# mfkiwl/msckf_stereo_c

Hardware: AMD Instinct MI355X
Metric: stereo frames/sec/node on EuRoC-shape input; ATE RMSE vs CPU ref (higher is better)
Workload: dtype f64

## Files before the change

### msckf_stereo_c_amd/csrc/abi/mskf_capi_ekf.cpp

```cpp
#include <algorithm>
#include <chrono>
#include <cmath>
#include <cstring>
#include "../../../include/mskf_chi2_table.h"
#include "mskf_internal.h"

namespace {
constexpr int kMaxRows = 65536;

size_t align_up(size_t v, size_t a) { return (v + a - 1) / a * a; }

int dev_alloc(double **p, size_t n, hipStream_t st) {
    MSKF_HIPCHK(hipMalloc((void **)p, n * sizeof(double)));
    MSKF_HIPCHK(hipMemsetAsync(*p, 0, n * sizeof(double), st));
    return MSKF_OK;
}
}

struct EkfExtra {
    EkfStreamDev desc_static;
    bool desc_valid = false;
    double *P_alt = nullptr;
    std::vector<double *> retired_hs;
};
// ... 377 lines not shown
    unsigned long long clone_mask = 0ULL;
    bool pairs = a.n_feat > 0, wave = a.n_feat > 0;
    int pair_a = -1, pair_b = -1, frows_cls[3] = {0, 0, 0};
    for (int j = 0; j < a.n_feat; ++j) {
        const mskf_ekf_feature &f = a.features[j];
        L.n_tri += f.needs_init ? 1 : 0;
        if (f.n_obs < 2 || f.n_obs > E.max_clones || f.obs_start < 0 || f.obs_start + f.n_obs > a.n_obs) return MSKF_ERR_INVALID;
        if (f.needs_init && (f.n_init < 1 || f.n_init > E.max_clones || f.init_start < 0 || f.init_start + f.n_init > a.n_obs)) return MSKF_ERR_INVALID;
        if (f.n_obs != 2) pairs = false;
        else if (pairs) {
            const int c0 = a.obs_clone[f.obs_start], c1 = a.obs_clone[f.obs_start + 1];
            if (j == 0) { pair_a = c0; pair_b = c1; }
            if (!(c0 < c1) || c0 != pair_a || c1 != pair_b) pairs = false;
        }
        if (f.n_obs > FEAT_WAVE_CLONES || (f.needs_init && f.n_init > TRI_SMALL_CLONES)) wave = false;
        L.m_total += 4 * f.n_obs - 3;
        B.max_frows = std::max(B.max_frows, 4 * f.n_obs);
        const int cls = std::max(f.n_obs, f.needs_init ? f.n_init : 0) <= FEAT_SMALL_CLONES ? 1 : 2;
        frows_cls[cls] = std::max(frows_cls[cls], 4 * f.n_obs);
        ++L.cnt[cls];
        for (int o = 0; o < f.n_obs; ++o) {
            const int c = a.obs_clone[f.obs_start + o];
            if (c < 0 || c >= a.n_clones) return MSKF_ERR_INVALID;
            clone_mask |= 1ULL << c;
        }
        const double nj = 4.0 * f.n_obs - 3.0, M = f.n_obs, dd = E.d;
        B.fl_feat += 2.0 * nj * (4.0 * M) * (6.0 * M) + 2.0 * nj * dd * dd + 2.0 * nj * nj * dd;
    }
    if (L.m_total > kMaxRows) { mskf_set_error("stacked Jacobian exceeds the row capacity"); return MSKF_ERR_CAPACITY; }
    L.clones = B.in_bytes;
    L.feats = align_up(L.clones + sizeof(mskf_clone_state) * (size_t)a.n_clones, 16);
    L.obs_clone = align_up(L.feats + sizeof(EkfFeatDev) * (size_t)a.n_feat, 16);
    L.obs_z = align_up(L.obs_clone + sizeof(int) * (size_t)a.n_obs, 16);
    L.tri = align_up(L.obs_z + sizeof(double) * 4 * (size_t)a.n_obs, 16);
// ... 71 lines not shown
        }
    for (int i = 0; i < n; ++i) {
        const mskf_ekf_update_args &a = args[i];
        const EkfUpdatePlan &L = plan[i];
        if (a.n_clones) std::memcpy(hin + L.clones, a.clones, sizeof(mskf_clone_state) * (size_t)a.n_clones);
        EkfFeatDev *fd = (EkfFeatDev *)(hin + L.feats);
        int *tri = (int *)(hin + L.tri);
        int n_tri_w = 0, row = 0;
        for (int j = 0; j < a.n_feat; ++j) {
            const mskf_ekf_feature &f = a.features[j];
            fd[j].obs_start = f.obs_start; fd[j].n_obs = f.n_obs;
            fd[j].needs_init = f.needs_init; fd[j].init_start = f.init_start; fd[j].n_init = f.n_init;
            fd[j].row_off = row;
            fd[j].position[0] = f.position[0]; fd[j].position[1] = f.position[1]; fd[j].position[2] = f.position[2];
            fd[j].colmask = 0ULL;
            row += 4 * f.n_obs - 3;
            if (f.needs_init) tri[n_tri_w++] = j;
        }
        if (a.n_obs) {
            std::memcpy(hin + L.obs_clone, a.obs_clone, sizeof(int) * (size_t)a.n_obs);
            std::memcpy(hin + L.obs_z, a.obs_z, sizeof(double) * 4 * (size_t)a.n_obs);
        }
        EkfStreamDev &D = ctx->ekf_desc.h[i];
        base_desc(streams[i], D);
        D.n_clones = a.n_clones; D.n_feat = a.n_feat; D.n_obs = a.n_obs;
        D.route = L.route; D.na_max = L.na_max;
        D.dof_offset = a.dof_offset; D.apply_row_cap = a.apply_row_cap;
        D.m_total = L.m_total;
        for (int k = 0; k < 3; ++k) D.gravity[k] = a.gravity[k];
        D.clones = (const mskf_clone_state *)(din + L.clones);
        D.feats = (EkfFeatDev *)(din + L.feats);
// ... 272 lines not shown
```

### msckf_stereo_c_amd/csrc/hip/ekf_cap.h

```cpp
#pragma once
#include "ekf_device.h"

struct EkfCapResult {
    int stacked;
    int end;
    int na;
    unsigned long long clones;
};

__device__ __forceinline__ int ekf_act_column(unsigned long long clones, int i) {
    int q = i / 6;
    unsigned long long m = clones;
    while (q-- > 0) m &= m - 1;
    return EKF_IMU_DIM + 6 * (int)__builtin_ctzll(m) + i % 6;
}

template <int NT = 256>
__device__ __forceinline__ EkfCapResult ekf_cap_local(const EkfStreamDev &S, bool publish) {
    __shared__ int s_sum[NT], s_cross[NT];
    __shared__ unsigned long long s_or[NT / 64];
    __shared__ int s_cap_from, s_tot[2];
    __shared__ unsigned long long s_mask;
    const int tid = threadIdx.x, nf = S.n_feat;
    const int per = (nf + NT - 1) / NT;
    const int j0 = tid * per, j1 = min(nf, j0 + per);
    __syncthreads();
    int local = 0;
    for (int j = j0; j < j1; ++j) if (S.feat_status[j] & 2) local += 4 * S.feats[j].n_obs - 3;
    s_sum[tid] = local;
    __syncthreads();
    for (int off = 1; off < NT; off <<= 1) {
        const int v = tid >= off ? s_sum[tid - off] : 0;
        __syncthreads();
        s_sum[tid] += v;
        __syncthreads();
    }
    const int before = s_sum[tid] - local;
    int cross = nf;
    if (S.apply_row_cap) {
        int run = before;
        for (int j = j0; j < j1; ++j)
            if (S.feat_status[j] & 2) { run += 4 * S.feats[j].n_obs - 3; if (run > S.max_stack_rows) { cross = j; break; } }
    }
    s_cross[tid] = cross;
    __syncthreads();
    if (tid == 0) {
        int c = nf;
        for (int t = 0; t < NT; ++t) if (s_cross[t] < c) c = s_cross[t];
        s_cap_from = c < nf ? c + 1 : nf;
    }
    __syncthreads();
    const int cap_from = s_cap_from;
    int stack = 0, meff = 0;
    unsigned long long orm = 0ULL;
    for (int j = j0; j < j1; ++j) {
        EkfFeatDev &F = S.feats[j];
        const int n = 4 * F.n_obs - 3;
        const bool pass = (S.feat_status[j] & 2) != 0;
        if (pass && j < cap_from) { stack += n; meff = F.row_off + n; orm |= F.colmask; }
        else if (pass && publish) {
            F.colmask = 0ULL; S.feat_status[j] &= (uint8_t)~2;
            for (int i = 0; i < n; ++i) S.rowmask[F.row_off + i] = 0ULL;
        }
    }
    __syncthreads();
    s_sum[tid] = stack; s_cross[tid] = meff;
    for (int off = 32; off > 0; off >>= 1) orm |= __shfl_xor(orm, off);
    if ((tid & 63) == 0) s_or[tid >> 6] = orm;
    __syncthreads();
    if (tid == 0) {
        int st = 0, me = 0;
        for (int t = 0; t < NT; ++t) { st += s_sum[t]; if (s_cross[t] > me) me = s_cross[t]; }
        unsigned long long m = 0ULL;
        for (int w = 0; w < NT / 64; ++w) m |= s_or[w];
// ... 19 lines not shown
```

### msckf_stereo_c_amd/csrc/hip/ekf_kernels.hip

```cpp
#include <mutex>
#include <type_traits>
#include "ekf_device.h"
#include "ekf_meas.h"
#include "chol_block.h"

using namespace ekf;

#define WG 256

__device__ __forceinline__ double wave_sum(double v) {
    for (int off = 32; off > 0; off >>= 1) v += __shfl_xor(v, off);
    return v;
}

__device__ __forceinline__ double block_sum(double v, double *s_red) {
    v = wave_sum(v);
    const int nw = blockDim.x >> 6;
    __syncthreads();
    if ((threadIdx.x & 63) == 0) s_red[threadIdx.x >> 6] = v;
    __syncthreads();
    double t = 0;
    for (int i = 0; i < nw; ++i) t += s_red[i];
    return t;
}
// ... 335 lines not shown

#define GATE_LDS_ROWS 120
__device__ __forceinline__ size_t pk(int i, int j) { return (size_t)i * (i + 1) / 2 + j; }
template <int MAXC, bool WAVE, int TPB>
__global__ __launch_bounds__(TPB, 2) void k_ekf_feature_blocks(const EkfStreamDev *streams, const int *work, int n_work, int lds_rows, int arena_doubles, int cls_lo, int cls_hi) {
    constexpr int GS = WAVE ? 64 : TPB;
    constexpr int NSUB = TPB / GS;
    const int gt = WAVE ? (int)(threadIdx.x & 63) : (int)threadIdx.x;
    const int sub = WAVE ? (int)(threadIdx.x >> 6) : 0;
    const int item = (int)blockIdx.x * NSUB + sub;
    if (item >= n_work) return;
    const int wcode = work[item];
    const int w_slot = (wcode >> 8) & 0xff, w_nslots = wcode & 0xff;
    const EkfStreamDev &S = streams[wcode >> 16];
    const int d = S.d, ld = S.ld;
    constexpr int BLK_DOUBLES = (12 + 24 + 4 + 12) * MAXC + 3 * (6 * MAXC + 1);
    constexpr int PAN_RS = WAVE ? 16 : ((4 * MAXC + 15) / 16) * 16;
    static_assert(WAVE || BLK_DOUBLES >= LNB * PAN_RS, "panel does not fit the dead scratch");
    __shared__ double s_blk_all[NSUB][BLK_DOUBLES];
    double *s_blk = s_blk_all[sub];
    double (*sHf)[3] = reinterpret_cast<double (*)[3]>(s_blk);
    double (*sHx)[6] = reinterpret_cast<double (*)[6]>(s_blk + 12 * MAXC);
    double *sr = s_blk + 36 * MAXC;
    double (*sV)[4 * MAXC] = reinterpret_cast<double (*)[4 * MAXC]>(s_blk + 40 * MAXC);
    double (*sCoef)[3] = reinterpret_cast<double (*)[3]>(s_blk + 52 * MAXC);
    __shared__ CholBlockShared s_cb;
    __shared__ double sBeta_all[NSUB][3], sVV_all[NSUB][3];
    __shared__ int sObsOfClone_all[NSUB][MAX_CLONES_DEV];
    __shared__ int sCloneOfObs_all[NSUB][MAXC];
    extern __shared__ double s_arena_all[];
    double *s_arena = s_arena_all + (size_t)sub * arena_doubles;
    typedef typename std::conditional<WAVE, TriScratchT<2 * TRI_SMALL_CLONES>,
                                      typename std::conditional<(MAXC <= FEAT_SMALL_CLONES), TriScratchT<2 * MAXC>, TriScratch>::type>::type TriT;
    TriT &sTri = *reinterpret_cast<TriT *>(s_arena);
    __shared__ double sW_all[NSUB][4 * MAXC];
    __shared__ double sRo_all[NSUB][4 * MAXC];
    __shared__ double sPos_all[NSUB][3];
    __shared__ int sValid_all[NSUB];
    __shared__ double sRed[8];
    double *sBeta = sBeta_all[sub], *sVV = sVV_all[sub], *sW = sW_all[sub], *sPos = sPos_all[sub], *sRo = sRo_all[sub];
    int *sObsOfClone = sObsOfClone_all[sub], *sCloneOfObs = sCloneOfObs_all[sub];
    int &sValid = sValid_all[sub];
    auto GSYNC = [&]() {
        if (WAVE) { __builtin_amdgcn_wave_barrier(); __builtin_amdgcn_s_waitcnt(0xc07f) ; asm volatile("" ::: "memory"); __builtin_amdgcn_wave_barrier(); }
        else __syncthreads();
    };
    auto gsum = [&](double v) { return WAVE ? wave_sum(v) : block_sum(v, sRed); };

    int ordinal = -1;
    for (int j = 0; j < S.n_feat; ++j) {
        EkfFeatDev &F = S.feats[j];
        {
            const int cls = F.needs_init && F.n_init > F.n_obs ? F.n_init : F.n_obs;
            if (cls < cls_lo || cls > cls_hi) continue;
            if (++ordinal % w_nslots != w_slot) continue;
        }
        GSYNC();
#ifdef FEAT_DBG
        long long tdbg[12]; int ndbg = 0;
#define TDBG() do { if (ndbg < 12) tdbg[ndbg++] = wall_clock64(); } while (0)
#else
#define TDBG() do {} while (0)
#endif
        TDBG();
        const int M = F.n_obs, rows = 4 * M, n = rows - 3;
        double *Hrow0 = S.Hs + (size_t)F.row_off * ld;
        if (gt < 64) {
            bool valid = true;
            double pos[3] = {F.position[0], F.position[1], F.position[2]};
            if (F.needs_init) valid = triangulate_wave(S, F, sTri, pos);
            if (gt == 0) {
                sPos[0] = pos[0]; sPos[1] = pos[1]; sPos[2] = pos[2];
                sValid = valid ? 1 : 0;
                F.position[0] = pos[0]; F.position[1] = pos[1]; F.position[2] = pos[2];
                S.pos_out[3 * j] = pos[0]; S.pos_out[3 * j + 1] = pos[1]; S.pos_out[3 * j + 2] = pos[2];
            }
        }
        for (int c = gt; c < MAX_CLONES_DEV; c += GS) sObsOfClone[c] = -1;
        GSYNC();
        if (!sValid || M < 2) {
            if (gt == 0) { S.feat_status[j] = 0; S.gamma[j] = -1.0; F.colmask = 0ULL; }
            for (int i = gt; i < n; i += GS) S.rowmask[F.row_off + i] = 0ULL;
            continue;
        }
        TDBG();
        if (gt < M) {
            const int o = F.obs_start + gt;
            const int ci = S.obs_clone[o];
            sObsOfClone[ci] = gt;
            sCloneOfObs[gt] = ci;
            const mskf_clone_state &cam = S.clones[ci];
            double R_w_c0[9], R_w_c1[9], t_c1_w[3], Rn[9], Hx[4][6], r[4];
            cam_pose(cam, S.R_c0_c1, S.t_c0_c1, R_w_c0, R_w_c1, t_c1_w, Rn);
            meas_jacobian(cam, R_w_c0, R_w_c1, t_c1_w, Rn, S.R_c0_c1, sPos, S.gravity, S.obs_z + 4 * o, Hx, r);
            for (int rr = 0; rr < 4; ++rr) for (int c = 0; c < 6; ++c) sHx[4 * gt + rr][c] = Hx[rr][c];
            for (int rr = 0; rr < 4; ++rr) for (int c = 0; c < 3; ++c) sHf[4 * gt + rr][c] = -sHx[4 * gt + rr][3 + c];
            for (int rr = 0; rr < 4; ++rr) sr[4 * gt + rr] = r[rr];
        }
        GSYNC();
        TDBG();
        for (int k = 0; k < 3; ++k) {
            double part = 0;
            for (int i = k + gt; i < rows; i += GS) part += sHf[i][k] * sHf[i][k];
            const double nrm2 = gsum(part);
            const double nrm = sqrt(nrm2);
            const double x0 = sHf[k][k];
            const double alpha = x0 > 0 ? -nrm : nrm;
            GSYNC();
            for (int i = gt; i < rows; i += GS) sV[k][i] = (i < k) ? 0.0 : (i == k ? x0 - alpha : sHf[i][k]);
            GSYNC();
            double pv = 0;
            for (int i = k + gt; i < rows; i += GS) pv += sV[k][i] * sV[k][i];
// ... 12 lines not shown
            double p21 = 0, p31 = 0, p32 = 0;
            for (int i = gt; i < rows; i += GS) { p21 += sV[1][i] * sV[0][i]; p31 += sV[2][i] * sV[0][i]; p32 += sV[2][i] * sV[1][i]; }
            const double a = gsum(p21), b = gsum(p31), c = gsum(p32);
            if (gt == 0) { sVV[0] = a; sVV[1] = b; sVV[2] = c; }
        }
        GSYNC();
        TDBG();
        {
            double r1 = 0, r2 = 0, r3 = 0;
            for (int i = gt; i < rows; i += GS) { const double rv = sr[i]; r1 += sV[0][i] * rv; r2 += sV[1][i] * rv; r3 += sV[2][i] * rv; }
            r1 = gsum(r1); r2 = gsum(r2); r3 = gsum(r3);
            for (int cc = gt; cc <= 6 * M; cc += GS) {
                double s1 = 0, s2 = 0, s3 = 0;
                if (cc < 6 * M) {
                    const int blk = cc / 6, c6 = cc - 6 * blk;
                    for (int rr = 0; rr < 4; ++rr) {
                        const double v = sHx[4 * blk + rr][c6];
                        s1 += sV[0][4 * blk + rr] * v; s2 += sV[1][4 * blk + rr] * v; s3 += sV[2][4 * blk + rr] * v;
                    }
                } else { s1 = r1; s2 = r2; s3 = r3; }
                const double c1 = sBeta[0] * s1;
                const double c2 = sBeta[1] * (s2 - c1 * sVV[0]);
                const double c3 = sBeta[2] * (s3 - c1 * sVV[1] - c2 * sVV[2]);
                sCoef[cc][0] = c1; sCoef[cc][1] = c2; sCoef[cc][2] = c3;
            }
        }
        GSYNC();
        TDBG();
        if constexpr (MAXC <= 32) {
            constexpr int NCH = (6 * MAXC + 63) / 64;
            double q0[NCH], q1[NCH], q2[NCH];
            int qcol[NCH], qob[NCH], qc6[NCH];
#pragma unroll
            for (int q = 0; q < NCH; ++q) {
                const int cc = (gt & 63) + 64 * q;
                qob[q] = -1; qcol[q] = 0; qc6[q] = 0; q0[q] = q1[q] = q2[q] = 0.0;
                if (cc < 6 * M) {
                    const int ob = cc / 6, c6 = cc - 6 * ob;
                    qob[q] = ob; qc6[q] = c6; qcol[q] = EKF_IMU_DIM + 6 * sCloneOfObs[ob] + c6;
                    q0[q] = sCoef[cc][0]; q1[q] = sCoef[cc][1]; q2[q] = sCoef[cc][2];
                }
            }
            for (int i = 3 + (gt >> 6); i < rows; i += GS / 64) {
                const double v0 = sV[0][i], v1 = sV[1][i], v2 = sV[2][i];
                double *out = Hrow0 + (size_t)(i - 3) * ld;
                const int ob_i = i >> 2;
#pragma unroll
                for (int q = 0; q < NCH; ++q) {
                    if (qob[q] < 0) continue;
                    const double base = (ob_i == qob[q]) ? sHx[i][qc6[q]] : 0.0;
                    out[qcol[q]] = base - q0[q] * v0 - q1[q] * v1 - q2[q] * v2;
                }
            }
        } else
        for (int i = 3 + (gt >> 6); i < rows; i += GS / 64) {
            const double v0 = sV[0][i], v1 = sV[1][i], v2 = sV[2][i];
            double *out = Hrow0 + (size_t)(i - 3) * ld;
            const int ob_i = i >> 2;
            for (int cc = gt & 63; cc < 6 * M; cc += 64) {
                const int ob = cc / 6, c6 = cc - 6 * ob;
                const double base = (ob_i == ob) ? sHx[i][c6] : 0.0;
                out[EKF_IMU_DIM + 6 * sCloneOfObs[ob] + c6] = base - sCoef[cc][0] * v0 - sCoef[cc][1] * v1 - sCoef[cc][2] * v2;
            }
        }
        for (int i = 3 + gt; i < rows; i += GS) {
            const double rv = sr[i] - sCoef[6 * M][0] * sV[0][i] - sCoef[6 * M][1] * sV[1][i] - sCoef[6 * M][2] * sV[2][i];
            sRo[i - 3] = rv;
            Hrow0[(size_t)(i - 3) * ld + d] = rv;
        }
        GSYNC();
        TDBG();
        auto gate_steps = [&](double *Mm) __attribute__((always_inline)) {
        const double *P = S.P;
        if constexpr (WAVE) {
            constexpr int NC = 6 * MAXC;
            static_assert(17 * 18 / 2 + 16 + 2 * (4 * MAXC - 3) * NC <= (int)(sizeof(TriScratchT<2 * TRI_SMALL_CLONES>) / 8), "H_o and H_o P_cc fit the arena behind the gate matrix");
            double *Ho = Mm + 17 * 18 / 2 + 16, *HP = Ho + (4 * MAXC - 3) * NC;
            const int nc = 6 * M;
            for (int e = gt; e < n * nc; e += GS) {
                const int i = e / nc + 3, cc = e - (i - 3) * nc;
                const int ob = cc / 6, c6 = cc - 6 * ob;
                const double base = ((i >> 2) == ob) ? sHx[i][c6] : 0.0;
                Ho[(i - 3) * NC + cc] = base - sCoef[cc][0] * sV[0][i] - sCoef[cc][1] * sV[1][i] - sCoef[cc][2] * sV[2][i];
            }
            GSYNC();
            for (int e = gt; e < n * nc; e += GS) {
                const int i = e / nc, v = e - i * nc;
                const int cv = EKF_IMU_DIM + 6 * sCloneOfObs[v / 6] + v % 6;
                double t = 0;
                for (int u = 0; u < nc; ++u) t += Ho[i * NC + u] * P[(size_t)(EKF_IMU_DIM + 6 * sCloneOfObs[u / 6] + u % 6) * ld + cv];
                HP[i * NC + v] = t;
            }
            GSYNC();
            for (int e = gt; e < n * n; e += GS) {
                const int i = e / n, k = e - i * n;
                if (k > i) continue;
                double t = 0;
                for (int v = 0; v < nc; ++v) t += HP[i * NC + v] * Ho[k * NC + v];
                Mm[pk(i + 3, k + 3)] = t;
            }
            GSYNC();
        } else {
        for (int pr = gt; pr < M * M; pr += GS) {
            const int a = pr / M, b = pr - a * M;
            if (b > a) continue;
            const int ca = EKF_IMU_DIM + 6 * sCloneOfObs[a], cb = EKF_IMU_DIM + 6 * sCloneOfObs[b];
            double Pab[6][6];
            for (int u = 0; u < 6; ++u) for (int v = 0; v < 6; ++v) Pab[u][v] = P[(size_t)(ca + u) * ld + cb + v];
            double HP[4][6];
            for (int i = 0; i < 4; ++i) for (int v = 0; v < 6; ++v) {
                double t = 0;
                for (int u = 0; u < 6; ++u) t += sHx[4 * a + i][u] * Pab[u][v];
                HP[i][v] = t;
            }
            for (int i = 0; i < 4; ++i) for (int jj = 0; jj < 4; ++jj) {
                if (a == b && jj > i) continue;
                double t = 0;
                for (int v = 0; v < 6; ++v) t += HP[i][v] * sHx[4 * b + jj][v];
                Mm[pk(4 * a + i, 4 * b + jj)] = t;
            }
        }
        GSYNC();
        TDBG();
        {
            double (*sWm)[3] = sHf;
            double (*sZ)[3] = sCoef;
            if (gt < rows) {
                const int i = gt;
                double w0 = 0, w1 = 0, w2 = 0;
                const double *mi = Mm + pk(i, 0);
#pragma unroll 4
                for (int c = 0; c <= i; ++c) { const double m = mi[c]; w0 += m * sV[0][c]; w1 += m * sV[1][c]; w2 += m * sV[2][c]; }
#pragma unroll 4
                for (int c = i + 1; c < rows; ++c) { const double m = Mm[pk(c, i)]; w0 += m * sV[0][c]; w1 += m * sV[1][c]; w2 += m * sV[2][c]; }
// ... 76 lines not shown
                GSYNC();
                for (int i = k + 1 + gt; i < n; i += GS) sW[i] -= SG(i, k) * yk;
            }
        }
#undef SG
        TDBG();
#ifdef FEAT_DBG
        if (item == 0 && gt == 0) printf("feat M=%d TPB=%d: tri %lld jac %lld hh %lld coef %lld write %lld gateM %lld reflect W %lld GZ %lld upd %lld chol %lld\n", M, TPB,
            (tdbg[1]-tdbg[0])*10, (tdbg[2]-tdbg[1])*10, (tdbg[3]-tdbg[2])*10, (tdbg[4]-tdbg[3])*10, (tdbg[5]-tdbg[4])*10, (tdbg[6]-tdbg[5])*10, (tdbg[7]-tdbg[6])*10,
            (tdbg[8]-tdbg[7])*10, (tdbg[9]-tdbg[8])*10, (tdbg[10]-tdbg[9])*10);
#endif
        double gamma = 1e300;
        if (pd_ok) {
            GSYNC();
            double pg = 0;
            for (int i = gt; i < n; i += GS) pg += sW[i] * sW[i];
            gamma = gsum(pg);
        }
        const int dof = M + S.dof_offset;
        const bool pass = pd_ok && dof >= 1 && dof < 100 && gamma < S.chi2[dof];
        if (gt < 64) {
            unsigned long long cm = 0ULL;
            if (pass) for (int o = gt; o < M; o += 64) cm |= 1ULL << sCloneOfObs[o];
            for (int off = 32; off > 0; off >>= 1) cm |= __shfl_xor(cm, off);
            for (int i = gt; i < n; i += 64) S.rowmask[F.row_off + i] = cm;
            if (gt == 0) { S.feat_status[j] = (uint8_t)(1 | (pass ? 2 : 0)); S.gamma[j] = gamma; F.colmask = cm; }
        }
        };
        if (rows <= lds_rows) gate_steps(s_arena);
        else gate_steps(S.gate_S + (size_t)w_slot * S.nmax * S.nmax);
    }
// ... 4 lines not shown
    if (!(S.route & EKF_ROUTE_PAIRS)) return;
    __shared__ TriScratch sTri;
    for (int t = blockIdx.x; t < S.n_tri; t += gridDim.x) {
        const int j = S.tri_idx[t];
        EkfFeatDev &F = S.feats[j];
        double pos[3] = {F.position[0], F.position[1], F.position[2]};
        __syncthreads();
        const bool valid = triangulate_wave(S, F, sTri, pos);
        if (threadIdx.x == 0) {
            F.position[0] = pos[0]; F.position[1] = pos[1]; F.position[2] = pos[2];
            S.feat_status[j] = valid ? 1 : 0;
        }
    }
}

#define PAIR_SLAB 153
__global__ __launch_bounds__(64) void k_ekf_pair_blocks(const EkfStreamDev *streams) {
    const EkfStreamDev &S = streams[blockIdx.y];
    if (!(S.route & EKF_ROUTE_PAIRS)) return;
    const int d = S.d, ld = S.ld;
    extern __shared__ double s_pair[];
    __shared__ double sPcc[12 * 12];
    __shared__ double sRw[2][2][9], sTc1[2][3], sRn[2][9];
    __shared__ int sPair[2];
    double *X = s_pair + (size_t)threadIdx.x * PAIR_SLAB;
    double *Hf = X + 104;
    double *V = Hf + 24;
    for (int base = blockIdx.x * 64; base < S.n_feat; base += gridDim.x * 64) {
        const int j = base + threadIdx.x;
        const bool have = j < S.n_feat;
        __syncthreads();
        if (threadIdx.x == 0) {
            const EkfFeatDev &F0 = S.feats[base];
            sPair[0] = S.obs_clone[F0.obs_start]; sPair[1] = S.obs_clone[F0.obs_start + 1];
        }
        __syncthreads();
        const int pa = sPair[0], pb = sPair[1];
        for (int e = threadIdx.x; e < 144; e += 64) {
            const int u = e / 12, v = e - 12 * u;
            const int cu = EKF_IMU_DIM + 6 * (u < 6 ? pa : pb) + (u % 6), cv = EKF_IMU_DIM + 6 * (v < 6 ? pa : pb) + (v % 6);
            sPcc[e] = S.P[(size_t)cu * ld + cv];
        }
// ... 1 lines not shown
            const mskf_clone_state &cam = S.clones[threadIdx.x == 0 ? pa : pb];
            double R0[9], R1[9], t1[3], Rn[9];
            cam_pose(cam, S.R_c0_c1, S.t_c0_c1, R0, R1, t1, Rn);
            for (int i = 0; i < 9; ++i) { sRw[threadIdx.x][0][i] = R0[i]; sRw[threadIdx.x][1][i] = R1[i]; sRn[threadIdx.x][i] = Rn[i]; }
            for (int i = 0; i < 3; ++i) sTc1[threadIdx.x][i] = t1[i];
        }
        __syncthreads();
        if (!have) continue;
        EkfFeatDev &F = S.feats[j];
        const int c0 = S.obs_clone[F.obs_start], c1 = S.obs_clone[F.obs_start + 1];
        const bool valid = F.needs_init ? (S.feat_status[j] & 1) != 0 : true;
        const double pos[3] = {F.position[0], F.position[1], F.position[2]};
        S.pos_out[3 * j] = pos[0]; S.pos_out[3 * j + 1] = pos[1]; S.pos_out[3 * j + 2] = pos[2];
        if (!valid || F.n_obs != 2 || c0 != pa || c1 != pb) {
            S.feat_status[j] = 0; S.gamma[j] = -1.0; F.colmask = 0ULL;
            for (int i = 0; i < 4 * F.n_obs - 3; ++i) S.rowmask[F.row_off + i] = 0ULL;
            continue;
        }
        for (int i = 0; i < 104; ++i) X[i] = 0.0;
        const double g[3] = {S.gravity[0], S.gravity[1], S.gravity[2]};
#pragma unroll 1
        for (int ob = 0; ob < 2; ++ob) {
            double Hx[4][6], r[4];
            meas_jacobian(S.clones[ob == 0 ? pa : pb], sRw[ob][0], sRw[ob][1], sTc1[ob], sRn[ob], S.R_c0_c1, pos, g, S.obs_z + 4 * (F.obs_start + ob), Hx, r);
#pragma unroll
            for (int rr = 0; rr < 4; ++rr) {
                double *Xr = X + (4 * ob + rr) * 13;
                for (int c = 0; c < 6; ++c) Xr[6 * ob + c] = Hx[rr][c];
                for (int c = 0; c < 3; ++c) Hf[(4 * ob + rr) * 3 + c] = -Hx[rr][3 + c];
                Xr[12] = r[rr];
            }
        }
#pragma unroll 1
        for (int k = 0; k < 3; ++k) {
            double nrm2 = 0;
            for (int i = k; i < 8; ++i) nrm2 += Hf[i * 3 + k] * Hf[i * 3 + k];
            const double nrm = sqrt(nrm2);
            const double x0 = Hf[k * 3 + k];
            const double alpha = x0 > 0 ? -nrm : nrm;
            double vn = 0;
            for (int i = 0; i < 8; ++i) {
                const double v = (i < k) ? 0.0 : (i == k ? x0 - alpha : Hf[i * 3 + k]);
                V[k * 8 + i] = v;
                vn += v * v;
            }
            const double beta = (nrm == 0.0 || vn == 0.0) ? 0.0 : 2.0 / vn;
            for (int c = k + 1; c < 3; ++c) {
                double sdot = 0;
                for (int i = k; i < 8; ++i) sdot += V[k * 8 + i] * Hf[i * 3 + c];
                sdot *= beta;
                for (int i = k; i < 8; ++i) Hf[i * 3 + c] -= sdot * V[k * 8 + i];
            }
#pragma unroll 1
            for (int c = 0; c < 13; ++c) {
                double sdot = 0;
                for (int i = k; i < 8; ++i) sdot += V[k * 8 + i] * X[i * 13 + c];
                sdot *= beta;
                for (int i = k; i < 8; ++i) X[i * 13 + c] -= sdot * V[k * 8 + i];
            }
        }
        double Sg[5][5];
        {
#pragma unroll 1
            for (int i = 0; i < 5; ++i) {
                double *hp = i < 3 ? X + 12 * i : Hf + 12 * (i - 3);
#pragma unroll 1
                for (int v = 0; v < 12; ++v) {
                    double t = 0;
                    for (int u2 = 0; u2 < 12; ++u2) t += X[(3 + i) * 13 + u2] * sPcc[u2 * 12 + v];
                    hp[v] = t;
                }
            }
#pragma unroll
            for (int i = 0; i < 5; ++i) {
                const double *hp = i < 3 ? X + 12 * i : Hf + 12 * (i - 3);
#pragma unroll
                for (int jj = 0; jj < 5; ++jj) {
                    if (jj > i) continue;
                    double t = 0;
#pragma unroll 1
                    for (int v = 0; v < 12; ++v) t += hp[v] * X[(3 + jj) * 13 + v];
                    Sg[i][jj] = t + (i == jj ? S.sigma2 : 0.0);
                }
            }
        }
        bool pd_ok = true;
        double y[5];
#pragma unroll
        for (int i = 0; i < 5; ++i) y[i] = X[(3 + i) * 13 + 12];
#pragma unroll
        for (int k = 0; k < 5; ++k) {
            const double dk = Sg[k][k];
            pd_ok = pd_ok && (dk > 0);
            const double inv = 1.0 / sqrt(dk > 0 ? dk : 1.0);
#pragma unroll
            for (int i = k; i < 5; ++i) Sg[i][k] *= inv;
            y[k] *= inv;
#pragma unroll
            for (int a = k + 1; a < 5; ++a) {
#pragma unroll
                for (int b = k + 1; b <= a; ++b) Sg[a][b] -= Sg[a][k] * Sg[b][k];
                y[a] -= Sg[a][k] * y[k];
            }
        }
        double gamma = 1e300;
        if (pd_ok) { gamma = 0; for (int i = 0; i < 5; ++i) gamma += y[i] * y[i]; }
        const int dof = 2 + S.dof_offset;
        const bool pass = pd_ok && dof >= 1 && dof < 100 && gamma < S.chi2[dof];
        double *Hrow0 = S.Hs + (size_t)F.row_off * ld;
        for (int i = 0; i < 5; ++i) {
            double *out = Hrow0 + (size_t)i * ld;
            for (int c = 0; c < 6; ++c) {
                out[EKF_IMU_DIM + 6 * pa + c] = X[(3 + i) * 13 + c];
                out[EKF_IMU_DIM + 6 * pb + c] = X[(3 + i) * 13 + 6 + c];
            }
            out[d] = X[(3 + i) * 13 + 12];
        }
        S.feat_status[j] = (uint8_t)(1 | (pass ? 2 : 0));
        S.gamma[j] = gamma;
        F.colmask = pass ? ((1ULL << pa) | (1ULL << pb)) : 0ULL;
        for (int i = 0; i < 5; ++i) S.rowmask[F.row_off + i] = F.colmask;
    }
}

extern "C" {
void ekf_launch_propagate(const EkfStreamDev *d, int n, hipStream_t st) { hipLaunchKernelGGL(k_ekf_propagate, dim3(1, n), dim3(WG), 0, st, d); }
void ekf_launch_remove_clone(const EkfStreamDev *d, int n, hipStream_t st) {
    hipLaunchKernelGGL(k_ekf_remove_clone, dim3(32, n), dim3(WG), 0, st, d);
}
void ekf_launch_features(const EkfStreamDev *d, const int *work_wave, int n_wave, const int *work_small, int n_small, const int *work_big, int n_big,
                         int max_rows, int max_rows_small, int big_clones, hipStream_t st) {
    const int packed_max = ((GATE_LDS_ROWS + 1) * (GATE_LDS_ROWS + 2) / 2 + 16) * (int)sizeof(double);
    const int tri_doubles = (int)((sizeof(TriScratchT<2 * TRI_SMALL_CLONES>) + 7) / 8);
    static std::once_flag attr_once;
    std::call_once(attr_once, [=]() {
        (void)hipFuncSetAttribute(reinterpret_cast<const void *>(k_ekf_feature_blocks<32, false, WG>), hipFuncAttributeMaxDynamicSharedMemorySize, packed_max);
        (void)hipFuncSetAttribute(reinterpret_cast<const void *>(k_ekf_feature_blocks<MAX_CLONES_DEV, false, WG>), hipFuncAttributeMaxDynamicSharedMemorySize, packed_max);
        (void)hipFuncSetAttribute(reinterpret_cast<const void *>(k_ekf_feature_blocks<FEAT_WAVE_CLONES, true, WG>), hipFuncAttributeMaxDynamicSharedMemorySize, 4 * tri_doubles * 8);
    });
    static_assert(4 * FEAT_WAVE_CLONES <= 16, "the WAVE variant's gate matrix and Cholesky panel hold 16 block rows (PAN_RS)");
    const int ALL = 1 << 30;
    if (n_wave > 0)
        hipLaunchKernelGGL((k_ekf_feature_blocks<FEAT_WAVE_CLONES, true, WG>), dim3((n_wave + 3) / 4), dim3(WG), (size_t)4 * tri_doubles * 8, st, d, work_wave, n_wave, 4 * FEAT_WAVE_CLONES, tri_doubles, 0, ALL);
    if (n_small > 0) {
        const int lr = max_rows_small;
        size_t lds = ((size_t)(lr + 1) * (lr + 2) / 2 + 16) * sizeof(double);
        if (lds < sizeof(TriScratchT<2 * FEAT_SMALL_CLONES>)) lds = sizeof(TriScratchT<2 * FEAT_SMALL_CLONES>);
        hipLaunchKernelGGL((k_ekf_feature_blocks<FEAT_SMALL_CLONES, false, 64>), dim3(n_small), dim3(64), lds, st, d, work_small, n_small, lr, 0, 0, FEAT_SMALL_CLONES);
    }
    if (n_big <= 0) return;
    const int lds_rows = max_rows <= GATE_LDS_ROWS ? max_rows : GATE_LDS_ROWS;
    size_t lds = ((size_t)(lds_rows + 1) * (lds_rows + 2) / 2 + 16) * sizeof(double);
    if (lds < sizeof(TriScratch)) lds = sizeof(TriScratch);
    if (big_clones <= 32) hipLaunchKernelGGL((k_ekf_feature_blocks<32, false, WG>), dim3(n_big), dim3(WG), lds, st, d, work_big, n_big, lds_rows, 0, FEAT_SMALL_CLONES + 1, ALL);
    else hipLaunchKernelGGL((k_ekf_feature_blocks<MAX_CLONES_DEV, false, WG>), dim3(n_big), dim3(WG), lds, st, d, work_big, n_big, lds_rows, 0, FEAT_SMALL_CLONES + 1, ALL);
}
void ekf_launch_pair_features(const EkfStreamDev *d, int n, int max_feat, int max_tri, hipStream_t st) {
    if (max_tri > 0) {
// ... 21 lines not shown
```

### msckf_stereo_c_amd/csrc/hip/ekf_limits.h

```cpp
#pragma once

#if defined(__HIPCC__)
#define EKF_HD __host__ __device__ __forceinline__
#else
#define EKF_HD inline
#endif

#define EKF_IMU_DIM 21

#define MAX_CLONES_DEV 64
#define FEAT_WAVE_CLONES 4
#define FEAT_SMALL_CLONES 16
#define TRI_SMALL_CLONES 32
#define SU_MAX_NA 24
#define MSKF_DIRECT_MAX_ROWS 6
static_assert(FEAT_WAVE_CLONES <= FEAT_SMALL_CLONES && FEAT_SMALL_CLONES <= TRI_SMALL_CLONES && TRI_SMALL_CLONES <= MAX_CLONES_DEV, "size classes nest");
static_assert(MAX_CLONES_DEV <= 64, "clone sets are 64-bit masks (EkfFeatDev::colmask, rowmask)");

#define EKF_GEMM_TILE 32
#define SU_CH 128
#define CHOL_LDS_MAX_ROWS 181
#define CHOL_PAN_RS 192
#define TQ_THREADS 512
#define TS_RB 16
#define TS_LPF 14
#define QR_BIAS_LIMIT 1e-6
EKF_HD int chol_class(int d) { return d - EKF_IMU_DIM + 1 <= CHOL_LDS_MAX_ROWS ? 0 : 1; }
EKF_HD int tsqr_class(int d) { return d - EKF_IMU_DIM + 1 <= 2 * (TQ_THREADS / 4) ? 0 : 1; }
EKF_HD bool trsm_l_fits(int n) { return n + TS_RB <= 16 * TS_LPF; }

enum { EKF_QR_AUTO = 0, EKF_QR_GRAM = 1, EKF_QR_HOUSEHOLDER = 2, EKF_QR_REFERENCE = 3 };
EKF_HD bool ekf_mode_direct(int qr_mode, int stacked, int na) { return (qr_mode == EKF_QR_AUTO || qr_mode == EKF_QR_REFERENCE) && stacked <= na; }
EKF_HD bool ekf_mode_householder(int qr_mode) { return qr_mode == EKF_QR_HOUSEHOLDER || qr_mode == EKF_QR_REFERENCE; }
EKF_HD bool ekf_mode_redo_householder(int qr_mode, bool gram_factor, bool bias) { return ekf_mode_householder(qr_mode) || (qr_mode == EKF_QR_AUTO && (!gram_factor || bias)); }

enum {
    EKF_ROWS_STACKED = 0,
    EKF_ROWS_END = 1,
    EKF_ROWS_NA = 2,
    EKF_ROWS_DIAG = 3,
    EKF_ROWS_NK = 4,
    EKF_ROWS_COUNT = 5
};
enum {
    EKF_DIAG_HOUSEHOLDER = 1,
// ... 11 lines not shown
```

### msckf_stereo_c_amd/csrc/hip/ekf_meas.h

```cpp
#pragma once
#include "../../../include/mskf_hip.h"

#if defined(__HIPCC__)
#define EM_FN __host__ __device__ __forceinline__
#else
#define EM_FN inline
#endif

namespace ekf {

EM_FN void quat_to_rot(const double *q, double *R) {
    const double x = q[0], y = q[1], z = q[2], w = q[3];
    const double a = 2 * w * w - 1, tw = 2 * w;
    R[0] = a + 2 * x * x;        R[1] = tw * z + 2 * x * y;   R[2] = -tw * y + 2 * x * z;
    R[3] = -tw * z + 2 * y * x;  R[4] = a + 2 * y * y;        R[5] = tw * x + 2 * y * z;
    R[6] = tw * y + 2 * z * x;   R[7] = -tw * x + 2 * z * y;  R[8] = a + 2 * z * z;
}
EM_FN void mat3_mul(const double *A, const double *B, double *C) {
    for (int i = 0; i < 3; ++i) for (int j = 0; j < 3; ++j) C[3 * i + j] = A[3 * i] * B[j] + A[3 * i + 1] * B[3 + j] + A[3 * i + 2] * B[6 + j];
}
EM_FN void mat3_vec(const double *A, const double *v, double *o) {
    for (int i = 0; i < 3; ++i) o[i] = A[3 * i] * v[0] + A[3 * i + 1] * v[1] + A[3 * i + 2] * v[2];
}
EM_FN void mat3t_vec(const double *A, const double *v, double *o) {
// ... 50 lines not shown
    }
}

EM_FN void meas_jacobian(const mskf_clone_state &cam, const double *R_w_c0, const double *R_w_c1, const double *t_c1_w, const double *Rn,
                         const double *R_c0_c1, const double *pos, const double *g, const double *z, double Hx[4][6], double r[4]) {
    double p_c0[3], p_c1[3], A[4][6];
    meas_cam_points(R_w_c0, R_w_c1, cam.p, t_c1_w, pos, p_c0, p_c1);
    meas_unprojected(R_w_c0, R_w_c1, R_c0_c1, p_c0, p_c1, A);
    meas_project(A, Rn, cam.p_null, pos, g, Hx);
    r[0] = z[0] - p_c0[0] / p_c0[2];
    r[1] = z[1] - p_c0[1] / p_c0[2];
    r[2] = z[2] - p_c1[0] / p_c1[2];
    r[3] = z[3] - p_c1[1] / p_c1[2];
}

}
#undef EM_FN
```

Measured before the change: 106,900.

## Compress per-observation stereo Jacobian from four rows to three via feature-block reflectors

Each observation's 4x6 stereo Jacobian gets a 3-step Householder reduction on its 4x3 feature block. Only 3 rows are stored; the leftover 4th residual component adds rho^2/sigma2 to the chi-square gate. This shrinks stacked Jacobian rows, shared-memory blocks, the pair-kernel slab and the Cholesky sizes by about a quarter, while row capping still uses nominal counts. Risk: the 4th reflected row's pose columns are dropped even though they need not be zero, so the filter update may differ from the reference.

New measurement: 108,500 (median of 6 runs). About the same (+1.5%).

```diff
diff --git a/msckf_stereo_c_amd/csrc/abi/mskf_capi_ekf.cpp b/msckf_stereo_c_amd/csrc/abi/mskf_capi_ekf.cpp
--- a/msckf_stereo_c_amd/csrc/abi/mskf_capi_ekf.cpp
+++ b/msckf_stereo_c_amd/csrc/abi/mskf_capi_ekf.cpp
@@ -415,10 +415,10 @@
             if (!(c0 < c1) || c0 != pair_a || c1 != pair_b) pairs = false;
         }
         if (f.n_obs > FEAT_WAVE_CLONES || (f.needs_init && f.n_init > TRI_SMALL_CLONES)) wave = false;
-        L.m_total += 4 * f.n_obs - 3;
-        B.max_frows = std::max(B.max_frows, 4 * f.n_obs);
+        L.m_total += ekf_rows_nominal(f.n_obs);
+        B.max_frows = std::max(B.max_frows, 3 * f.n_obs);
         const int cls = std::max(f.n_obs, f.needs_init ? f.n_init : 0) <= FEAT_SMALL_CLONES ? 1 : 2;
-        frows_cls[cls] = std::max(frows_cls[cls], 4 * f.n_obs);
+        frows_cls[cls] = std::max(frows_cls[cls], 3 * f.n_obs);
         ++L.cnt[cls];
         for (int o = 0; o < f.n_obs; ++o) {
             const int c = a.obs_clone[f.obs_start + o];
@@ -520,7 +520,7 @@
             fd[j].row_off = row;
             fd[j].position[0] = f.position[0]; fd[j].position[1] = f.position[1]; fd[j].position[2] = f.position[2];
             fd[j].colmask = 0ULL;
-            row += 4 * f.n_obs - 3;
+            row += ekf_rows_stored(f.n_obs);
             if (f.needs_init) tri[n_tri_w++] = j;
         }
         if (a.n_obs) {
diff --git a/msckf_stereo_c_amd/csrc/hip/ekf_cap.h b/msckf_stereo_c_amd/csrc/hip/ekf_cap.h
--- a/msckf_stereo_c_amd/csrc/hip/ekf_cap.h
+++ b/msckf_stereo_c_amd/csrc/hip/ekf_cap.h
@@ -26,7 +26,7 @@
     const int j0 = tid * per, j1 = min(nf, j0 + per);
     __syncthreads();
     int local = 0;
-    for (int j = j0; j < j1; ++j) if (S.feat_status[j] & 2) local += 4 * S.feats[j].n_obs - 3;
+    for (int j = j0; j < j1; ++j) if (S.feat_status[j] & 2) local += ekf_rows_nominal(S.feats[j].n_obs);
     s_sum[tid] = local;
     __syncthreads();
     for (int off = 1; off < NT; off <<= 1) {
@@ -40,7 +40,7 @@
     if (S.apply_row_cap) {
         int run = before;
         for (int j = j0; j < j1; ++j)
-            if (S.feat_status[j] & 2) { run += 4 * S.feats[j].n_obs - 3; if (run > S.max_stack_rows) { cross = j; break; } }
+            if (S.feat_status[j] & 2) { run += ekf_rows_nominal(S.feats[j].n_obs); if (run > S.max_stack_rows) { cross = j; break; } }
     }
     s_cross[tid] = cross;
     __syncthreads();
@@ -55,9 +55,9 @@
     unsigned long long orm = 0ULL;
     for (int j = j0; j < j1; ++j) {
         EkfFeatDev &F = S.feats[j];
-        const int n = 4 * F.n_obs - 3;
+        const int n = ekf_rows_stored(F.n_obs);
         const bool pass = (S.feat_status[j] & 2) != 0;
-        if (pass && j < cap_from) { stack += n; meff = F.row_off + n; orm |= F.colmask; }
+        if (pass && j < cap_from) { stack += ekf_rows_nominal(F.n_obs); meff = F.row_off + n; orm |= F.colmask; }
         else if (pass && publish) {
             F.colmask = 0ULL; S.feat_status[j] &= (uint8_t)~2;
             for (int i = 0; i < n; ++i) S.rowmask[F.row_off + i] = 0ULL;
diff --git a/msckf_stereo_c_amd/csrc/hip/ekf_kernels.hip b/msckf_stereo_c_amd/csrc/hip/ekf_kernels.hip
--- a/msckf_stereo_c_amd/csrc/hip/ekf_kernels.hip
+++ b/msckf_stereo_c_amd/csrc/hip/ekf_kernels.hip
@@ -373,16 +373,16 @@
     const int w_slot = (wcode >> 8) & 0xff, w_nslots = wcode & 0xff;
     const EkfStreamDev &S = streams[wcode >> 16];
     const int d = S.d, ld = S.ld;
-    constexpr int BLK_DOUBLES = (12 + 24 + 4 + 12) * MAXC + 3 * (6 * MAXC + 1);
-    constexpr int PAN_RS = WAVE ? 16 : ((4 * MAXC + 15) / 16) * 16;
+    constexpr int BLK_DOUBLES = (9 + 18 + 3 + 9) * MAXC + 3 * (6 * MAXC + 1);
+    constexpr int PAN_RS = WAVE ? 16 : ((3 * MAXC + 15) / 16) * 16;
     static_assert(WAVE || BLK_DOUBLES >= LNB * PAN_RS, "panel does not fit the dead scratch");
     __shared__ double s_blk_all[NSUB][BLK_DOUBLES];
     double *s_blk = s_blk_all[sub];
     double (*sHf)[3] = reinterpret_cast<double (*)[3]>(s_blk);
-    double (*sHx)[6] = reinterpret_cast<double (*)[6]>(s_blk + 12 * MAXC);
-    double *sr = s_blk + 36 * MAXC;
-    double (*sV)[4 * MAXC] = reinterpret_cast<double (*)[4 * MAXC]>(s_blk + 40 * MAXC);
-    double (*sCoef)[3] = reinterpret_cast<double (*)[3]>(s_blk + 52 * MAXC);
+    double (*sHx)[6] = reinterpret_cast<double (*)[6]>(s_blk + 9 * MAXC);
+    double *sr = s_blk + 27 * MAXC;
+    double (*sV)[3 * MAXC] = reinterpret_cast<double (*)[3 * MAXC]>(s_blk + 30 * MAXC);
+    double (*sCoef)[3] = reinterpret_cast<double (*)[3]>(s_blk + 39 * MAXC);
     __shared__ CholBlockShared s_cb;
     __shared__ double sBeta_all[NSUB][3], sVV_all[NSUB][3];
     __shared__ int sObsOfClone_all[NSUB][MAX_CLONES_DEV];
@@ -393,7 +393,7 @@
                                       typename std::conditional<(MAXC <= FEAT_SMALL_CLONES), TriScratchT<2 * MAXC>, TriScratch>::type>::type TriT;
     TriT &sTri = *reinterpret_cast<TriT *>(s_arena);
     __shared__ double sW_all[NSUB][4 * MAXC];
-    __shared__ double sRo_all[NSUB][4 * MAXC];
+    __shared__ double sRo_all[NSUB][3 * MAXC];
     __shared__ double sPos_all[NSUB][3];
     __shared__ int sValid_all[NSUB];
     __shared__ double sRed[8];
@@ -422,7 +422,7 @@
 #define TDBG() do {} while (0)
 #endif
         TDBG();
-        const int M = F.n_obs, rows = 4 * M, n = rows - 3;
+        const int M = F.n_obs, rows = 3 * M, n = rows - 3;
         double *Hrow0 = S.Hs + (size_t)F.row_off * ld;
         if (gt < 64) {
             bool valid = true;
@@ -449,12 +449,14 @@
             sObsOfClone[ci] = gt;
             sCloneOfObs[gt] = ci;
             const mskf_clone_state &cam = S.clones[ci];
-            double R_w_c0[9], R_w_c1[9], t_c1_w[3], Rn[9], Hx[4][6], r[4];
+            double R_w_c0[9], R_w_c1[9], t_c1_w[3], Rn[9], Hx[4][6], r[4], Hx3[3][6], r3[3], rho;
             cam_pose(cam, S.R_c0_c1, S.t_c0_c1, R_w_c0, R_w_c1, t_c1_w, Rn);
             meas_jacobian(cam, R_w_c0, R_w_c1, t_c1_w, Rn, S.R_c0_c1, sPos, S.gravity, S.obs_z + 4 * o, Hx, r);
-            for (int rr = 0; rr < 4; ++rr) for (int c = 0; c < 6; ++c) sHx[4 * gt + rr][c] = Hx[rr][c];
-            for (int rr = 0; rr < 4; ++rr) for (int c = 0; c < 3; ++c) sHf[4 * gt + rr][c] = -sHx[4 * gt + rr][3 + c];
-            for (int rr = 0; rr < 4; ++rr) sr[4 * gt + rr] = r[rr];
+            meas_reduce_rank3(Hx, r, Hx3, r3, &rho);
+            for (int rr = 0; rr < 3; ++rr) for (int c = 0; c < 6; ++c) sHx[3 * gt + rr][c] = Hx3[rr][c];
+            for (int rr = 0; rr < 3; ++rr) for (int c = 0; c < 3; ++c) sHf[3 * gt + rr][c] = -sHx[3 * gt + rr][3 + c];
+            for (int rr = 0; rr < 3; ++rr) sr[3 * gt + rr] = r3[rr];
+            sW[n + gt] = rho;
         }
         GSYNC();
         TDBG();
@@ -497,9 +499,9 @@
                 double s1 = 0, s2 = 0, s3 = 0;
                 if (cc < 6 * M) {
                     const int blk = cc / 6, c6 = cc - 6 * blk;
-                    for (int rr = 0; rr < 4; ++rr) {
-                        const double v = sHx[4 * blk + rr][c6];
-                        s1 += sV[0][4 * blk + rr] * v; s2 += sV[1][4 * blk + rr] * v; s3 += sV[2][4 * blk + rr] * v;
+                    for (int rr = 0; rr < 3; ++rr) {
+                        const double v = sHx[3 * blk + rr][c6];
+                        s1 += sV[0][3 * blk + rr] * v; s2 += sV[1][3 * blk + rr] * v; s3 += sV[2][3 * blk + rr] * v;
                     }
                 } else { s1 = r1; s2 = r2; s3 = r3; }
                 const double c1 = sBeta[0] * s1;
@@ -527,7 +529,7 @@
             for (int i = 3 + (gt >> 6); i < rows; i += GS / 64) {
                 const double v0 = sV[0][i], v1 = sV[1][i], v2 = sV[2][i];
                 double *out = Hrow0 + (size_t)(i - 3) * ld;
-                const int ob_i = i >> 2;
+                const int ob_i = i / 3;
 #pragma unroll
                 for (int q = 0; q < NCH; ++q) {
                     if (qob[q] < 0) continue;
@@ -539,7 +541,7 @@
         for (int i = 3 + (gt >> 6); i < rows; i += GS / 64) {
             const double v0 = sV[0][i], v1 = sV[1][i], v2 = sV[2][i];
             double *out = Hrow0 + (size_t)(i - 3) * ld;
-            const int ob_i = i >> 2;
+            const int ob_i = i / 3;
             for (int cc = gt & 63; cc < 6 * M; cc += 64) {
                 const int ob = cc / 6, c6 = cc - 6 * ob;
                 const double base = (ob_i == ob) ? sHx[i][c6] : 0.0;
@@ -557,13 +559,13 @@
         const double *P = S.P;
         if constexpr (WAVE) {
             constexpr int NC = 6 * MAXC;
-            static_assert(17 * 18 / 2 + 16 + 2 * (4 * MAXC - 3) * NC <= (int)(sizeof(TriScratchT<2 * TRI_SMALL_CLONES>) / 8), "H_o and H_o P_cc fit the arena behind the gate matrix");
-            double *Ho = Mm + 17 * 18 / 2 + 16, *HP = Ho + (4 * MAXC - 3) * NC;
+            static_assert(17 * 18 / 2 + 16 + 2 * (3 * MAXC - 3) * NC <= (int)(sizeof(TriScratchT<2 * TRI_SMALL_CLONES>) / 8), "H_o and H_o P_cc fit the arena behind the gate matrix");
+            double *Ho = Mm + 17 * 18 / 2 + 16, *HP = Ho + (3 * MAXC - 3) * NC;
             const int nc = 6 * M;
             for (int e = gt; e < n * nc; e += GS) {
                 const int i = e / nc + 3, cc = e - (i - 3) * nc;
                 const int ob = cc / 6, c6 = cc - 6 * ob;
-                const double base = ((i >> 2) == ob) ? sHx[i][c6] : 0.0;
+                const double base = (i / 3 == ob) ? sHx[i][c6] : 0.0;
                 Ho[(i - 3) * NC + cc] = base - sCoef[cc][0] * sV[0][i] - sCoef[cc][1] * sV[1][i] - sCoef[cc][2] * sV[2][i];
             }
             GSYNC();
@@ -590,17 +592,17 @@
             const int ca = EKF_IMU_DIM + 6 * sCloneOfObs[a], cb = EKF_IMU_DIM + 6 * sCloneOfObs[b];
             double Pab[6][6];
             for (int u = 0; u < 6; ++u) for (int v = 0; v < 6; ++v) Pab[u][v] = P[(size_t)(ca + u) * ld + cb + v];
-            double HP[4][6];
-            for (int i = 0; i < 4; ++i) for (int v = 0; v < 6; ++v) {
+            double HP[3][6];
+            for (int i = 0; i < 3; ++i) for (int v = 0; v < 6; ++v) {
                 double t = 0;
-                for (int u = 0; u < 6; ++u) t += sHx[4 * a + i][u] * Pab[u][v];
+                for (int u = 0; u < 6; ++u) t += sHx[3 * a + i][u] * Pab[u][v];
                 HP[i][v] = t;
             }
-            for (int i = 0; i < 4; ++i) for (int jj = 0; jj < 4; ++jj) {
+            for (int i = 0; i < 3; ++i) for (int jj = 0; jj < 3; ++jj) {
                 if (a == b && jj > i) continue;
                 double t = 0;
-                for (int v = 0; v < 6; ++v) t += HP[i][v] * sHx[4 * b + jj][v];
-                Mm[pk(4 * a + i, 4 * b + jj)] = t;
+                for (int v = 0; v < 6; ++v) t += HP[i][v] * sHx[3 * b + jj][v];
+                Mm[pk(3 * a + i, 3 * b + jj)] = t;
             }
         }
         GSYNC();
@@ -707,7 +709,7 @@
         if (pd_ok) {
             GSYNC();
             double pg = 0;
-            for (int i = gt; i < n; i += GS) pg += sW[i] * sW[i];
+            for (int i = gt; i < n + M; i += GS) pg += i < n ? sW[i] * sW[i] : sW[i] * sW[i] / S.sigma2;
             gamma = gsum(pg);
         }
         const int dof = M + S.dof_offset;
@@ -742,7 +744,7 @@
     }
 }
 
-#define PAIR_SLAB 153
+#define PAIR_SLAB 115
 __global__ __launch_bounds__(64) void k_ekf_pair_blocks(const EkfStreamDev *streams) {
     const EkfStreamDev &S = streams[blockIdx.y];
     if (!(S.route & EKF_ROUTE_PAIRS)) return;
@@ -752,8 +754,8 @@
     __shared__ double sRw[2][2][9], sTc1[2][3], sRn[2][9];
     __shared__ int sPair[2];
     double *X = s_pair + (size_t)threadIdx.x * PAIR_SLAB;
-    double *Hf = X + 104;
-    double *V = Hf + 24;
+    double *Hf = X + 78;
+    double *V = Hf + 18;
     for (int base = blockIdx.x * 64; base < S.n_feat; base += gridDim.x * 64) {
         const int j = base + threadIdx.x;
         const bool have = j < S.n_feat;
@@ -785,56 +787,59 @@
         S.pos_out[3 * j] = pos[0]; S.pos_out[3 * j + 1] = pos[1]; S.pos_out[3 * j + 2] = pos[2];
         if (!valid || F.n_obs != 2 || c0 != pa || c1 != pb) {
             S.feat_status[j] = 0; S.gamma[j] = -1.0; F.colmask = 0ULL;
-            for (int i = 0; i < 4 * F.n_obs - 3; ++i) S.rowmask[F.row_off + i] = 0ULL;
+            for (int i = 0; i < ekf_rows_stored(F.n_obs); ++i) S.rowmask[F.row_off + i] = 0ULL;
             continue;
         }
-        for (int i = 0; i < 104; ++i) X[i] = 0.0;
+        for (int i = 0; i < 78; ++i) X[i] = 0.0;
         const double g[3] = {S.gravity[0], S.gravity[1], S.gravity[2]};
+        double rho2 = 0;
 #pragma unroll 1
         for (int ob = 0; ob < 2; ++ob) {
-            double Hx[4][6], r[4];
+            double Hx[4][6], r[4], Hx3[3][6], r3[3], rho;
             meas_jacobian(S.clones[ob == 0 ? pa : pb], sRw[ob][0], sRw[ob][1], sTc1[ob], sRn[ob], S.R_c0_c1, pos, g, S.obs_z + 4 * (F.obs_start + ob), Hx, r);
-#pragma unroll
-            for (int rr = 0; rr < 4; ++rr) {
-                double *Xr = X + (4 * ob + rr) * 13;
-                for (int c = 0; c < 6; ++c) Xr[6 * ob + c] = Hx[rr][c];
-                for (int c = 0; c < 3; ++c) Hf[(4 * ob + rr) * 3 + c] = -Hx[rr][3 + c];
-                Xr[12] = r[rr];
+            meas_reduce_rank3(Hx, r, Hx3, r3, &rho);
+            rho2 += rho * rho;
+#pragma unroll
+            for (int rr = 0; rr < 3; ++rr) {
+                double *Xr = X + (3 * ob + rr) * 13;
+                for (int c = 0; c < 6; ++c) Xr[6 * ob + c] = Hx3[rr][c];
+                for (int c = 0; c < 3; ++c) Hf[(3 * ob + rr) * 3 + c] = -Hx3[rr][3 + c];
+                Xr[12] = r3[rr];
             }
         }
 #pragma unroll 1
         for (int k = 0; k < 3; ++k) {
             double nrm2 = 0;
-            for (int i = k; i < 8; ++i) nrm2 += Hf[i * 3 + k] * Hf[i * 3 + k];
+            for (int i = k; i < 6; ++i) nrm2 += Hf[i * 3 + k] * Hf[i * 3 + k];
             const double nrm = sqrt(nrm2);
             const double x0 = Hf[k * 3 + k];
             const double alpha = x0 > 0 ? -nrm : nrm;
             double vn = 0;
-            for (int i = 0; i < 8; ++i) {
+            for (int i = 0; i < 6; ++i) {
                 const double v = (i < k) ? 0.0 : (i == k ? x0 - alpha : Hf[i * 3 + k]);
-                V[k * 8 + i] = v;
+                V[k * 6 + i] = v;
                 vn += v * v;
             }
             const double beta = (nrm == 0.0 || vn == 0.0) ? 0.0 : 2.0 / vn;
             for (int c = k + 1; c < 3; ++c) {
                 double sdot = 0;
-                for (int i = k; i < 8; ++i) sdot += V[k * 8 + i] * Hf[i * 3 + c];
+                for (int i = k; i < 6; ++i) sdot += V[k * 6 + i] * Hf[i * 3 + c];
                 sdot *= beta;
-                for (int i = k; i < 8; ++i) Hf[i * 3 + c] -= sdot * V[k * 8 + i];
+                for (int i = k; i < 6; ++i) Hf[i * 3 + c] -= sdot * V[k * 6 + i];
             }
 #pragma unroll 1
             for (int c = 0; c < 13; ++c) {
                 double sdot = 0;
-                for (int i = k; i < 8; ++i) sdot += V[k * 8 + i] * X[i * 13 + c];
+                for (int i = k; i < 6; ++i) sdot += V[k * 6 + i] * X[i * 13 + c];
                 sdot *= beta;
-                for (int i = k; i < 8; ++i) X[i * 13 + c] -= sdot * V[k * 8 + i];
-            }
-        }
-        double Sg[5][5];
+                for (int i = k; i < 6; ++i) X[i * 13 + c] -= sdot * V[k * 6 + i];
+            }
+        }
+        double Sg[3][3];
         {
 #pragma unroll 1
-            for (int i = 0; i < 5; ++i) {
-                double *hp = i < 3 ? X + 12 * i : Hf + 12 * (i - 3);
+            for (int i = 0; i < 3; ++i) {
+                double *hp = X + 12 * i;
 #pragma unroll 1
                 for (int v = 0; v < 12; ++v) {
                     double t = 0;
@@ -843,10 +848,10 @@
                 }
             }
 #pragma unroll
-            for (int i = 0; i < 5; ++i) {
-                const double *hp = i < 3 ? X + 12 * i : Hf + 12 * (i - 3);
-#pragma unroll
-                for (int jj = 0; jj < 5; ++jj) {
+            for (int i = 0; i < 3; ++i) {
+                const double *hp = X + 12 * i;
+#pragma unroll
+                for (int jj = 0; jj < 3; ++jj) {
                     if (jj > i) continue;
                     double t = 0;
 #pragma unroll 1
@@ -856,30 +861,30 @@
             }
         }
         bool pd_ok = true;
-        double y[5];
-#pragma unroll
-        for (int i = 0; i < 5; ++i) y[i] = X[(3 + i) * 13 + 12];
-#pragma unroll
-        for (int k = 0; k < 5; ++k) {
+        double y[3];
+#pragma unroll
+        for (int i = 0; i < 3; ++i) y[i] = X[(3 + i) * 13 + 12];
+#pragma unroll
+        for (int k = 0; k < 3; ++k) {
             const double dk = Sg[k][k];
             pd_ok = pd_ok && (dk > 0);
             const double inv = 1.0 / sqrt(dk > 0 ? dk : 1.0);
 #pragma unroll
-            for (int i = k; i < 5; ++i) Sg[i][k] *= inv;
+            for (int i = k; i < 3; ++i) Sg[i][k] *= inv;
             y[k] *= inv;
 #pragma unroll
-            for (int a = k + 1; a < 5; ++a) {
+            for (int a = k + 1; a < 3; ++a) {
 #pragma unroll
                 for (int b = k + 1; b <= a; ++b) Sg[a][b] -= Sg[a][k] * Sg[b][k];
                 y[a] -= Sg[a][k] * y[k];
             }
         }
         double gamma = 1e300;
-        if (pd_ok) { gamma = 0; for (int i = 0; i < 5; ++i) gamma += y[i] * y[i]; }
+        if (pd_ok) { gamma = 0; for (int i = 0; i < 3; ++i) gamma += y[i] * y[i]; gamma += rho2 / S.sigma2; }
         const int dof = 2 + S.dof_offset;
         const bool pass = pd_ok && dof >= 1 && dof < 100 && gamma < S.chi2[dof];
         double *Hrow0 = S.Hs + (size_t)F.row_off * ld;
-        for (int i = 0; i < 5; ++i) {
+        for (int i = 0; i < 3; ++i) {
             double *out = Hrow0 + (size_t)i * ld;
             for (int c = 0; c < 6; ++c) {
                 out[EKF_IMU_DIM + 6 * pa + c] = X[(3 + i) * 13 + c];
@@ -890,7 +895,7 @@
         S.feat_status[j] = (uint8_t)(1 | (pass ? 2 : 0));
         S.gamma[j] = gamma;
         F.colmask = pass ? ((1ULL << pa) | (1ULL << pb)) : 0ULL;
-        for (int i = 0; i < 5; ++i) S.rowmask[F.row_off + i] = F.colmask;
+        for (int i = 0; i < 3; ++i) S.rowmask[F.row_off + i] = F.colmask;
     }
 }
 
@@ -909,10 +914,10 @@
         (void)hipFuncSetAttribute(reinterpret_cast<const void *>(k_ekf_feature_blocks<MAX_CLONES_DEV, false, WG>), hipFuncAttributeMaxDynamicSharedMemorySize, packed_max);
         (void)hipFuncSetAttribute(reinterpret_cast<const void *>(k_ekf_feature_blocks<FEAT_WAVE_CLONES, true, WG>), hipFuncAttributeMaxDynamicSharedMemorySize, 4 * tri_doubles * 8);
     });
-    static_assert(4 * FEAT_WAVE_CLONES <= 16, "the WAVE variant's gate matrix and Cholesky panel hold 16 block rows (PAN_RS)");
+    static_assert(3 * FEAT_WAVE_CLONES <= 16, "the WAVE variant's gate matrix and Cholesky panel hold 16 block rows (PAN_RS)");
     const int ALL = 1 << 30;
     if (n_wave > 0)
-        hipLaunchKernelGGL((k_ekf_feature_blocks<FEAT_WAVE_CLONES, true, WG>), dim3((n_wave + 3) / 4), dim3(WG), (size_t)4 * tri_doubles * 8, st, d, work_wave, n_wave, 4 * FEAT_WAVE_CLONES, tri_doubles, 0, ALL);
+        hipLaunchKernelGGL((k_ekf_feature_blocks<FEAT_WAVE_CLONES, true, WG>), dim3((n_wave + 3) / 4), dim3(WG), (size_t)4 * tri_doubles * 8, st, d, work_wave, n_wave, 3 * FEAT_WAVE_CLONES, tri_doubles, 0, ALL);
     if (n_small > 0) {
         const int lr = max_rows_small;
         size_t lds = ((size_t)(lr + 1) * (lr + 2) / 2 + 16) * sizeof(double);
diff --git a/msckf_stereo_c_amd/csrc/hip/ekf_limits.h b/msckf_stereo_c_amd/csrc/hip/ekf_limits.h
--- a/msckf_stereo_c_amd/csrc/hip/ekf_limits.h
+++ b/msckf_stereo_c_amd/csrc/hip/ekf_limits.h
@@ -29,6 +29,9 @@
 EKF_HD int tsqr_class(int d) { return d - EKF_IMU_DIM + 1 <= 2 * (TQ_THREADS / 4) ? 0 : 1; }
 EKF_HD bool trsm_l_fits(int n) { return n + TS_RB <= 16 * TS_LPF; }
 
+EKF_HD int ekf_rows_nominal(int n_obs) { return 4 * n_obs - 3; }
+EKF_HD int ekf_rows_stored(int n_obs) { return 3 * n_obs - 3; }
+
 enum { EKF_QR_AUTO = 0, EKF_QR_GRAM = 1, EKF_QR_HOUSEHOLDER = 2, EKF_QR_REFERENCE = 3 };
 EKF_HD bool ekf_mode_direct(int qr_mode, int stacked, int na) { return (qr_mode == EKF_QR_AUTO || qr_mode == EKF_QR_REFERENCE) && stacked <= na; }
 EKF_HD bool ekf_mode_householder(int qr_mode) { return qr_mode == EKF_QR_HOUSEHOLDER || qr_mode == EKF_QR_REFERENCE; }
diff --git a/msckf_stereo_c_amd/csrc/hip/ekf_meas.h b/msckf_stereo_c_amd/csrc/hip/ekf_meas.h
--- a/msckf_stereo_c_amd/csrc/hip/ekf_meas.h
+++ b/msckf_stereo_c_amd/csrc/hip/ekf_meas.h
@@ -4,6 +4,7 @@
 #if defined(__HIPCC__)
 #define EM_FN __host__ __device__ __forceinline__
 #else
+#include <math.h>
 #define EM_FN inline
 #endif
 
@@ -88,5 +89,58 @@
     r[3] = z[3] - p_c1[1] / p_c1[2];
 }
 
+EM_FN double meas_sumsq4(const double v[4]) {
+    double s = 0, c = 0;
+    for (int i = 0; i < 4; ++i) {
+        const double p = v[i] * v[i], e = fma(v[i], v[i], -p);
+        const double t = s + p, bb = t - s;
+        c += ((s - (t - bb)) + (p - bb)) + e;
+        s = t;
+    }
+    return s + c;
+}
+EM_FN void meas_rank3_reflectors(double Hf[4][3], double v[3][4], double beta[3]) {
+    for (int k = 0; k < 3; ++k) {
+        double nrm2 = 0;
+        for (int i = k; i < 4; ++i) nrm2 += Hf[i][k] * Hf[i][k];
+        const double nrm = sqrt(nrm2);
+        const double x0 = Hf[k][k];
+        const double alpha = x0 > 0 ? -nrm : nrm;
+        for (int i = 0; i < 4; ++i) v[k][i] = i < k ? 0.0 : (i == k ? x0 - alpha : Hf[i][k]);
+        const double vn = meas_sumsq4(v[k]);
+        beta[k] = (nrm == 0.0 || vn == 0.0) ? 0.0 : 2.0 / vn;
+        for (int c = k + 1; c < 3; ++c) {
+            double s = 0;
+            for (int i = k; i < 4; ++i) s += v[k][i] * Hf[i][c];
+            s *= beta[k];
+            for (int i = k; i < 4; ++i) Hf[i][c] -= s * v[k][i];
+        }
+        Hf[k][k] = beta[k] == 0.0 ? x0 : alpha;
+        for (int i = k + 1; i < 4; ++i) Hf[i][k] = beta[k] == 0.0 ? Hf[i][k] : 0.0;
+    }
+}
+EM_FN void meas_rank3_apply(const double v[3][4], const double beta[3], double x[4]) {
+    for (int k = 0; k < 3; ++k) {
+        double s = 0;
+        for (int i = k; i < 4; ++i) s += v[k][i] * x[i];
+        s *= beta[k];
+        for (int i = k; i < 4; ++i) x[i] -= s * v[k][i];
+    }
+}
+EM_FN void meas_reduce_rank3(const double Hx[4][6], const double r[4], double Hx3[3][6], double r3[3], double *rho) {
+    double Hf[4][3], v[3][4], beta[3], x[4];
+    for (int i = 0; i < 4; ++i) for (int c = 0; c < 3; ++c) Hf[i][c] = -Hx[i][3 + c];
+    meas_rank3_reflectors(Hf, v, beta);
+    for (int c = 0; c < 3; ++c) {
+        for (int i = 0; i < 4; ++i) x[i] = Hx[i][c];
+        meas_rank3_apply(v, beta, x);
+        for (int i = 0; i < 3; ++i) { Hx3[i][c] = x[i]; Hx3[i][3 + c] = -Hf[i][c]; }
+    }
+    for (int i = 0; i < 4; ++i) x[i] = r[i];
+    meas_rank3_apply(v, beta, x);
+    for (int i = 0; i < 3; ++i) r3[i] = x[i];
+    *rho = x[3];
+}
+
 }
 #undef EM_FN
```
